# pothosware/PothosComms

Measured on AMD Instinct MI355X. Metric: Msamples/s complex_float32 255-tap FIR, higher is better.
Workload: dtype f32

## Files before the change

### pothoscomms_amd/csrc/fft4096.hpp

```cpp
#pragma once
#include <hip/hip_runtime.h>

namespace pcx {
namespace fft4k {

constexpr int N = 4096;
constexpr int T = 256;
constexpr int LDS_DATA = N + N / 16;
constexpr int LDS_TW2 = 15 * 16;
constexpr int LDS_ELEMS = LDS_DATA + LDS_TW2;
constexpr int TW_TABLE_ELEMS = 15 * 16 + 15 * 256;

typedef float cf __attribute__((ext_vector_type(2)));

__device__ __forceinline__ void cmul2(cf &a, cf &b, cf wa, cf wb)
{
    cf ra, rb;
    asm("v_pk_mul_f32 %0, %2, %4 op_sel:[1,1] op_sel_hi:[0,1] neg_lo:[0,1]\n\t"
        "v_pk_mul_f32 %1, %3, %5 op_sel:[1,1] op_sel_hi:[0,1] neg_lo:[0,1]\n\t"
        "v_pk_fma_f32 %0, %2, %4, %0 op_sel:[0,0,0] op_sel_hi:[1,0,1]\n\t"
        "v_pk_fma_f32 %1, %3, %5, %1 op_sel:[0,0,0] op_sel_hi:[1,0,1]"
        : "=&v"(ra), "=&v"(rb)
        : "v"(a), "v"(b), "v"(wa), "v"(wb));
    a = ra;
    b = rb;
}
__device__ __forceinline__ void cmul2_conj(cf &a, cf &b, cf ha, cf hb)
{
    cf ra, rb;
    asm("v_pk_mul_f32 %0, %2, %4 op_sel:[1,1] op_sel_hi:[0,1] neg_lo:[0,1] neg_hi:[0,1]\n\t"
        "v_pk_mul_f32 %1, %3, %5 op_sel:[1,1] op_sel_hi:[0,1] neg_lo:[0,1] neg_hi:[0,1]\n\t"
        "v_pk_fma_f32 %0, %2, %4, %0 op_sel:[0,0,0] op_sel_hi:[1,0,1] neg_hi:[1,0,0]\n\t"
        "v_pk_fma_f32 %1, %3, %5, %1 op_sel:[0,0,0] op_sel_hi:[1,0,1] neg_hi:[1,0,0]"
        : "=&v"(ra), "=&v"(rb)
        : "v"(a), "v"(b), "v"(ha), "v"(hb));
    a = ra;
    b = rb;
}
__device__ __forceinline__ void addsub_mi(cf &p, cf &m, cf a, cf d)
{
    asm("v_pk_add_f32 %0, %2, %3 op_sel:[0,1] op_sel_hi:[1,0] neg_hi:[0,1]\n\t"
        "v_pk_add_f32 %1, %2, %3 op_sel:[0,1] op_sel_hi:[1,0] neg_lo:[0,1]"
        : "=&v"(p), "=&v"(m)
        : "v"(a), "v"(d));
}
__device__ __forceinline__ cf cmul_cs(cf a, float c, float s)
{
    return cf{__builtin_fmaf(a.x, c, a.y * s), __builtin_fmaf(a.y, c, -a.x * s)};
}

__device__ __forceinline__ void fft4(cf &a0, cf &a1, cf &a2, cf &a3)
{
    const cf t0 = a0 + a2, t1 = a0 - a2, t2 = a1 + a3, d = a1 - a3;
    a0 = t0 + t2;
    a2 = t0 - t2;
    addsub_mi(a1, a3, t1, d);
}
__device__ __forceinline__ void fft4_mi2(cf &a0, cf &a1, cf &a2, cf &a3)
{
    cf t0, t1;
    addsub_mi(t0, t1, a0, a2);
    const cf t2 = a1 + a3, d = a1 - a3;
    a0 = t0 + t2;
    a2 = t0 - t2;
    addsub_mi(a1, a3, t1, d);
}

__device__ __forceinline__ void fft4_conj(cf &a0, cf &a1, cf &a2, cf &a3)
{
    const cf t0 = a0 + a2, t1 = a0 - a2, t2 = a1 + a3, d = a1 - a3;
    asm("v_pk_add_f32 %0, %4, %5 neg_hi:[1,1]\n\t"
        "v_pk_add_f32 %1, %4, %5 neg_lo:[0,1] neg_hi:[1,0]\n\t"
        "v_pk_add_f32 %2, %6, %7 op_sel:[0,1] op_sel_hi:[1,0] neg_hi:[1,0]\n\t"
        "v_pk_add_f32 %3, %6, %7 op_sel:[0,1] op_sel_hi:[1,0] neg_lo:[0,1] neg_hi:[1,1]"
        : "=&v"(a0), "=&v"(a2), "=&v"(a1), "=&v"(a3)
        : "v"(t0), "v"(t2), "v"(t1), "v"(d));
}

struct LaneTw {
    cf a[3];
    cf c[12];
};

__device__ __forceinline__ void fft16_inner(cf (&v)[16])
{
#pragma unroll
    for (int n2 = 0; n2 < 4; n2++) fft4(v[n2], v[4 + n2], v[8 + n2], v[12 + n2]);
}
__device__ __forceinline__ void fft16_outer(cf (&v)[16])
{
#pragma unroll
    for (int k1 = 0; k1 < 4; k1++) fft4(v[4 * k1], v[4 * k1 + 1], v[4 * k1 + 2], v[4 * k1 + 3]);
}
__device__ __forceinline__ void fft16_plain(cf (&v)[16])
{
    constexpr float C1 = 0.92387953251128673848f;
    constexpr float S1 = 0.38268343236508978178f;
    constexpr float R2 = 0.70710678118654752440f;
    fft16_inner(v);
    v[4 * 1 + 1] = cmul_cs(v[4 * 1 + 1], C1, S1);
    v[4 * 1 + 2] = cmul_cs(v[4 * 1 + 2], R2, R2);
    v[4 * 1 + 3] = cmul_cs(v[4 * 1 + 3], S1, C1);
    v[4 * 2 + 1] = cmul_cs(v[4 * 2 + 1], R2, R2);
    v[4 * 2 + 3] = cmul_cs(v[4 * 2 + 3], -R2, R2);
    v[4 * 3 + 1] = cmul_cs(v[4 * 3 + 1], S1, C1);
    v[4 * 3 + 2] = cmul_cs(v[4 * 3 + 2], -R2, R2);
    v[4 * 3 + 3] = cmul_cs(v[4 * 3 + 3], -C1, -S1);
    fft4(v[0], v[1], v[2], v[3]);
    fft4(v[4], v[5], v[6], v[7]);
    fft4_mi2(v[8], v[9], v[10], v[11]);
    fft4(v[12], v[13], v[14], v[15]);
}
__device__ __forceinline__ void fft16_tw(cf (&v)[16], const LaneTw &tw)
{
#pragma unroll
    for (int n1 = 1; n1 < 4; n1++) {
        cmul2(v[4 * n1 + 0], v[4 * n1 + 1], tw.a[n1 - 1], tw.a[n1 - 1]);
        cmul2(v[4 * n1 + 2], v[4 * n1 + 3], tw.a[n1 - 1], tw.a[n1 - 1]);
    }
    fft16_inner(v);
#pragma unroll
    for (int n2 = 1; n2 < 4; n2++) {
        cmul2(v[4 * 0 + n2], v[4 * 1 + n2], tw.c[(n2 - 1) * 4 + 0], tw.c[(n2 - 1) * 4 + 1]);
        cmul2(v[4 * 2 + n2], v[4 * 3 + n2], tw.c[(n2 - 1) * 4 + 2], tw.c[(n2 - 1) * 4 + 3]);
    }
    fft16_outer(v);
}
__device__ __forceinline__ void fft16_tw_conj(cf (&v)[16], const LaneTw &tw)
{
#pragma unroll
    for (int n1 = 1; n1 < 4; n1++) {
        cmul2(v[4 * n1 + 0], v[4 * n1 + 1], tw.a[n1 - 1], tw.a[n1 - 1]);
        cmul2(v[4 * n1 + 2], v[4 * n1 + 3], tw.a[n1 - 1], tw.a[n1 - 1]);
    }
    fft16_inner(v);
#pragma unroll
    for (int n2 = 1; n2 < 4; n2++) {
        cmul2(v[4 * 0 + n2], v[4 * 1 + n2], tw.c[(n2 - 1) * 4 + 0], tw.c[(n2 - 1) * 4 + 1]);
        cmul2(v[4 * 2 + n2], v[4 * 3 + n2], tw.c[(n2 - 1) * 4 + 2], tw.c[(n2 - 1) * 4 + 3]);
    }
#pragma unroll
    for (int k1 = 0; k1 < 4; k1++) fft4_conj(v[4 * k1], v[4 * k1 + 1], v[4 * k1 + 2], v[4 * k1 + 3]);
}
__device__ __forceinline__ constexpr int bin_of(int q) { return (q >> 2) + 4 * (q & 3); }

__device__ __forceinline__ void load_pass3_twiddles(LaneTw &t, const float2 *__restrict__ tab, int j)
{
    const cf *tb = reinterpret_cast<const cf *>(tab) + LDS_TW2;
#pragma unroll
    for (int p = 0; p < 3; p++) t.a[p] = tb[p * 256 + j];
#pragma unroll
    for (int p = 0; p < 12; p++) t.c[p] = tb[(3 + p) * 256 + j];
}
__device__ __forceinline__ void stage_pass2_twiddles(cf *lds, const float2 *__restrict__ tab, int j)
{
    if (j < LDS_TW2) lds[LDS_DATA + j] = reinterpret_cast<const cf *>(tab)[j];
}

typedef unsigned int u32x2 __attribute__((ext_vector_type(2)));

__device__ __forceinline__ __amdgpu_buffer_rsrc_t make_rsrc(const void *p, unsigned bytes)
{
    const unsigned long long a = reinterpret_cast<unsigned long long>(p);
    const unsigned lo = __builtin_amdgcn_readfirstlane((unsigned)a);
    const unsigned hi = __builtin_amdgcn_readfirstlane((unsigned)(a >> 32));
    return __builtin_amdgcn_make_buffer_rsrc(reinterpret_cast<void *>(((unsigned long long)hi << 32) | lo), 0,
                                             (int)__builtin_amdgcn_readfirstlane(bytes), 0x00020000);
}
constexpr int kAuxStream = 2;
template <bool CHECKED, int AUX = kAuxStream>
__device__ __forceinline__ void load_frame(cf (&v)[16], __amdgpu_buffer_rsrc_t rs, int j)
{
#pragma unroll
    for (int r = 0; r < 16; r++) {
        const u32x2 t = CHECKED ? __builtin_amdgcn_raw_buffer_load_b64(rs, (j + 256 * r) * 8, 0, AUX)
                                : __builtin_amdgcn_raw_buffer_load_b64(rs, j * 8, 2048 * r, AUX);
        v[r] = cf{__uint_as_float(t.x), __uint_as_float(t.y)};
    }
}
template <int AUX = 0>
__device__ __forceinline__ void store_cf(__amdgpu_buffer_rsrc_t rs, unsigned voff, cf a)
{
    u32x2 t;
    t.x = __float_as_uint(a.x);
    t.y = __float_as_uint(a.y);
    __builtin_amdgcn_raw_buffer_store_b64(t, rs, (int)voff, 0, AUX);
}

__device__ __forceinline__ cf load_cf(__amdgpu_buffer_rsrc_t rs, int voff, int soff)
{
    const u32x2 t = __builtin_amdgcn_raw_buffer_load_b64(rs, voff, soff, 0);
    return cf{__uint_as_float(t.x), __uint_as_float(t.y)};
}
__device__ __forceinline__ void load_pass3_twiddles(LaneTw &t, __amdgpu_buffer_rsrc_t tab, int j)
{
#pragma unroll
    for (int p = 0; p < 3; p++) t.a[p] = load_cf(tab, j * 8, (LDS_TW2 + p * 256) * 8);
#pragma unroll
    for (int p = 0; p < 12; p++) t.c[p] = load_cf(tab, j * 8, (LDS_TW2 + (3 + p) * 256) * 8);
}

__device__ __forceinline__ float fast_atan2f(float y, float x)
{
    const float ax = __builtin_fabsf(x), ay = __builtin_fabsf(y);
    const float mx = __builtin_fmaxf(ax, ay), mn = __builtin_fminf(ax, ay);
    const float t = mx > 0.f ? mn * __builtin_amdgcn_rcpf(mx) : 0.f;
    const float s = t * t;
    float p = 0.006811532657593489f;
    p = __builtin_fmaf(p, s, -0.03360334783792496f);
    p = __builtin_fmaf(p, s, 0.0796225368976593f);
    p = __builtin_fmaf(p, s, -0.1323327124118805f);
    p = __builtin_fmaf(p, s, 0.19807793200016022f);
    p = __builtin_fmaf(p, s, -0.3331736624240875f);
    p = __builtin_fmaf(p, s, 0.9999961256980896f);
    float r = t * p;
    r = ay > ax ? 1.57079632679489661923f - r : r;
    r = (__float_as_uint(x) >> 31) ? 3.14159265358979323846f - r : r;
    return __builtin_copysignf(r, y);
}

__device__ __forceinline__ cf fast_atan2f_x2(cf y, cf x)
{
    const cf ax = {__builtin_fabsf(x.x), __builtin_fabsf(x.y)}, ay = {__builtin_fabsf(y.x), __builtin_fabsf(y.y)};
    const cf mx = {__builtin_fmaxf(ax.x, ay.x), __builtin_fmaxf(ax.y, ay.y)};
    const cf mn = {__builtin_fminf(ax.x, ay.x), __builtin_fminf(ax.y, ay.y)};
    const cf rc = {mx.x > 0.f ? __builtin_amdgcn_rcpf(mx.x) : 0.f, mx.y > 0.f ? __builtin_amdgcn_rcpf(mx.y) : 0.f};
    const cf t = mn * rc;
    const cf s = t * t;
    auto k2 = [](float c) { return cf{c, c}; };
    cf p = k2(0.006811532657593489f);
    p = __builtin_elementwise_fma(p, s, k2(-0.03360334783792496f));
    p = __builtin_elementwise_fma(p, s, k2(0.0796225368976593f));
    p = __builtin_elementwise_fma(p, s, k2(-0.1323327124118805f));
    p = __builtin_elementwise_fma(p, s, k2(0.19807793200016022f));
    p = __builtin_elementwise_fma(p, s, k2(-0.3331736624240875f));
    p = __builtin_elementwise_fma(p, s, k2(0.9999961256980896f));
    cf r = t * p;
    const cf ro = k2(1.57079632679489661923f) - r;
    r = cf{ay.x > ax.x ? ro.x : r.x, ay.y > ax.y ? ro.y : r.y};
    const cf rn = k2(3.14159265358979323846f) - r;
    r = cf{(__float_as_uint(x.x) >> 31) ? rn.x : r.x, (__float_as_uint(x.y) >> 31) ? rn.y : r.y};
    return cf{__builtin_copysignf(r.x, y.x), __builtin_copysignf(r.y, y.y)};
}

__device__ __forceinline__ int padi(int i) { return i + (i >> 4); }
__device__ __forceinline__ cf cmul1(cf a, cf w)
{
    cf t, r;
    asm("v_pk_mul_f32 %0, %2, %3 op_sel:[1,1] op_sel_hi:[0,1] neg_lo:[0,1]\n\t"
        "v_pk_fma_f32 %1, %2, %3, %0 op_sel:[0,0,0] op_sel_hi:[1,0,1]"
        : "=&v"(t), "=&v"(r)
        : "v"(a), "v"(w));
    return r;
}
__device__ __forceinline__ void fft8(cf &a0, cf &a1, cf &a2, cf &a3, cf &a4, cf &a5, cf &a6, cf &a7)
{
    constexpr float R2 = 0.70710678118654752440f;
    cf e0 = a0, e1 = a2, e2 = a4, e3 = a6, o0 = a1, o1 = a3, o2 = a5, o3 = a7;
    fft4(e0, e1, e2, e3);
    fft4(o0, o1, o2, o3);
    const cf w1 = cmul_cs(o1, R2, R2);
    const cf w3 = cmul_cs(o3, -R2, R2);
    cf p2, m2;
    addsub_mi(p2, m2, e2, o2);
    a0 = e0 + o0; a4 = e0 - o0;
    a1 = e1 + w1; a5 = e1 - w1;
    a2 = p2;      a6 = m2;
    a3 = e3 + w3; a7 = e3 - w3;
}

__device__ __forceinline__ void lds_barrier()
{
    __builtin_amdgcn_fence(__ATOMIC_RELEASE, "workgroup", "local");
    __builtin_amdgcn_s_barrier();
    __builtin_amdgcn_fence(__ATOMIC_ACQUIRE, "workgroup", "local");
}

template <int PART = 0>
__device__ __forceinline__ void pass1_math(cf (&v)[16])
{
    if (PART != 2) fft16_plain(v);
}
template <int PART = 0>
__device__ __forceinline__ void pass1_exchange(cf (&v)[16], cf *lds, int j)
{
    if (PART == 1) return;
    lds_barrier();
#pragma unroll
    for (int q = 0; q < 16; q++) lds[17 * j + bin_of(q)] = v[q];
}
template <int PART = 0>
__device__ __forceinline__ void pass1(cf (&v)[16], cf *lds, int j)
{
    pass1_math<PART>(v);
    pass1_exchange<PART>(v, lds, j);
}
template <int PART = 0>
__device__ __forceinline__ void pass2(cf (&v)[16], cf *lds, int j)
{
    if (PART != 1) {
        lds_barrier();
        const int rb = j + (j >> 4);
#pragma unroll
        for (int r = 0; r < 16; r++) v[r] = lds[rb + 272 * r];
    }
    LaneTw tw;
    const cf *t2 = lds + LDS_DATA + (j & 15);
#pragma unroll
    for (int p = 0; p < 3; p++) tw.a[p] = t2[p * 16];
#pragma unroll
    for (int p = 0; p < 12; p++) tw.c[p] = t2[(3 + p) * 16];
    if (PART != 2) fft16_tw(v, tw);
    else v[0] = v[0] + tw.a[0] + tw.c[0];
    if (PART == 1) return;
    lds_barrier();
    const int wb = (j >> 4) * 272 + (j & 15);
#pragma unroll
    for (int q = 0; q < 16; q++) lds[wb + 17 * bin_of(q)] = v[q];
}
template <int PART = 0, bool CONJ = false>
__device__ __forceinline__ void pass3(cf (&v)[16], const cf *lds, int j, const LaneTw &tw3)
{
    if (PART != 1) {
        lds_barrier();
        const int rb = j + (j >> 4);
#pragma unroll
        for (int r = 0; r < 16; r++) v[r] = lds[rb + 272 * r];
    }
    if (PART != 2) {
        if (CONJ) fft16_tw_conj(v, tw3);
        else fft16_tw(v, tw3);
    }
}

__device__ __forceinline__ void fft16_post(cf (&v)[16], const LaneTw &tw)
{
    fft16_inner(v);
#pragma unroll
    for (int k1 = 1; k1 < 4; k1++) {
        cmul2(v[4 * k1 + 0], v[4 * k1 + 1], tw.c[(k1 - 1) * 4 + 0], tw.c[(k1 - 1) * 4 + 1]);
        cmul2(v[4 * k1 + 2], v[4 * k1 + 3], tw.c[(k1 - 1) * 4 + 2], tw.c[(k1 - 1) * 4 + 3]);
    }
    fft16_outer(v);
#pragma unroll
    for (int k2 = 1; k2 < 4; k2++) {
        cmul2(v[4 * 0 + k2], v[4 * 1 + k2], tw.a[k2 - 1], tw.a[k2 - 1]);
        cmul2(v[4 * 2 + k2], v[4 * 3 + k2], tw.a[k2 - 1], tw.a[k2 - 1]);
    }
}
__device__ __forceinline__ void wave_lds_order()
{
    __builtin_amdgcn_fence(__ATOMIC_RELEASE, "wavefront", "local");
    __builtin_amdgcn_wave_barrier();
    __builtin_amdgcn_fence(__ATOMIC_ACQUIRE, "wavefront", "local");
}
__device__ __forceinline__ int spec_lane(int j) { return (j >> 4) + 16 * (j & 15); }
struct SpectrumLoad {
    cf row[16];
    cf tw2;
};
__device__ __forceinline__ void spectrum_request(SpectrumLoad &t, const float2 *__restrict__ spec, const float2 *__restrict__ twtab, int j)
{
    const __amdgpu_buffer_rsrc_t rs = make_rsrc(spec, N * 8);
#pragma unroll
    for (int k = 0; k < 16; k++) t.row[k] = load_cf(rs, j * 8, 2048 * k);
    t.tw2 = load_cf(make_rsrc(twtab, LDS_TW2 * 8), j * 8, 0);
}
__device__ __forceinline__ void spectrum_turn(cf (&H)[16], const SpectrumLoad &t, cf *lds, int j)
{
#pragma unroll
    for (int k = 0; k < 16; k++) lds[j + 272 * k] = t.row[k];
    if (j < LDS_TW2) lds[LDS_DATA + j] = t.tw2;
    lds_barrier();
#pragma unroll
    for (int k = 0; k < 16; k++) H[k] = lds[spec_lane(j) + 272 * k];
}
__device__ __forceinline__ void load_spectrum_lanes(cf (&H)[16], const float2 *__restrict__ spec, const float2 *__restrict__ twtab, cf *lds, int j)
{
    SpectrumLoad t;
    spectrum_request(t, spec, twtab, j);
    spectrum_turn(H, t, lds, j);
}
__device__ __forceinline__ void load_pass2_twiddles(LaneTw &tw, const cf *lds, int j)
{
    const cf *t2 = lds + LDS_DATA + (j & 15);
#pragma unroll
    for (int p = 0; p < 3; p++) tw.a[p] = t2[p * 16];
#pragma unroll
    for (int p = 0; p < 12; p++) tw.c[p] = t2[(3 + p) * 16];
}
__device__ __forceinline__ void dif_a_math(cf (&v)[16], const LaneTw &tw3) { fft16_post(v, tw3); }
struct NoHook { __device__ __forceinline__ void operator()() const {} };
template <typename HOOK = NoHook>
__device__ __forceinline__ void dif_rest(cf (&v)[16], cf *lds, int j, HOOK before_last = HOOK())
{
    const int row = 272 * (j >> 4), l = j & 15;
    lds_barrier();
#pragma unroll
    for (int q = 0; q < 16; q++) lds[j + 272 * bin_of(q)] = v[q];
    lds_barrier();
#pragma unroll
    for (int r = 0; r < 16; r++) v[r] = lds[row + l + 16 * r];
    LaneTw tw2;
    load_pass2_twiddles(tw2, lds, j);
    fft16_post(v, tw2);
    wave_lds_order();
#pragma unroll
    for (int q = 0; q < 16; q++) lds[row + l + 17 * bin_of(q)] = v[q];
    wave_lds_order();
#pragma unroll
    for (int r = 0; r < 16; r++) v[r] = lds[row + 17 * l + r];
    before_last();
    fft16_plain(v);
}
template <bool CONJ = true>
__device__ __forceinline__ void dit_back(cf (&u)[16], cf *lds, int j, const LaneTw &tw3)
{
    const int row = 272 * (j >> 4), l = j & 15;
    fft16_plain(u);
    wave_lds_order();
#pragma unroll
    for (int q = 0; q < 16; q++) lds[row + 17 * l + bin_of(q)] = u[q];
    wave_lds_order();
#pragma unroll
    for (int r = 0; r < 16; r++) u[r] = lds[row + l + 17 * r];
    LaneTw tw2;
    load_pass2_twiddles(tw2, lds, j);
    fft16_tw(u, tw2);
    wave_lds_order();
#pragma unroll
    for (int q = 0; q < 16; q++) lds[row + l + 16 * bin_of(q)] = u[q];
    lds_barrier();
#pragma unroll
    for (int r = 0; r < 16; r++) u[r] = lds[j + 272 * r];
    if (CONJ) fft16_tw_conj(u, tw3);
    else fft16_tw(u, tw3);
}

}
}
```

### pothoscomms_amd/csrc/fir_ols.hip

```cpp
#include "fft4096.hpp"
#include "ols_block.hpp"
#include "ols_geometry.hpp"
#include "pcx_sched.hpp"
#include <cstdio>
#include <cstdlib>

#include <type_traits>

#include "pcx_internal.hpp"

namespace pcx {

template <bool PREFETCH, int LAUX = 0, int SAUX = 0, int CHUNKED = 0, int DIAG = 0, bool HGLOBAL = false, bool GATED = false, int XCH = 0>
__global__ __launch_bounds__(256, (PREFETCH && !HGLOBAL) ? 3 : 4) void fir_cf32_ols4096_kernel(const float2 *__restrict__ in, size_t in_elems,
                                                                  float2 *__restrict__ out, size_t n_out,
                                                                  const float2 *__restrict__ Hspec, int Kov, int pad,
                                                                  const float2 *__restrict__ twtab, size_t first_full,
                                                                  size_t nfull, size_t nblocks, SchedState *__restrict__ sched, Gate gate)
{
    using namespace fft4k;
    __shared__ cf lds[LDS_ELEMS];
    const int j = threadIdx.x;
    const size_t S = (size_t)(N - Kov);
    size_t b, bend, bstep;
    __shared__ unsigned sched_slot;
    BlockDealer deal;
    if (CHUNKED == 3) {
        static_assert(CHUNKED != 3 || !PREFETCH, "the register prefetch needs the next block's index a block early");
        if (!deal.begin(sched, &sched_slot, nblocks, j)) { deal.finish(j); return; }
        b = GATED ? nblocks - 1 - deal.block() : deal.block();
        bend = nblocks; bstep = 0;
    } else if (CHUNKED == 2) {
        const size_t per = (nblocks + 7) / 8, x = blockIdx.x & 7;
        b = x * per + (blockIdx.x >> 3);
        bend = (x + 1) * per < nblocks ? (x + 1) * per : nblocks;
        bstep = gridDim.x >> 3;
    } else if (CHUNKED) {
        const size_t q = nblocks / gridDim.x, rem = nblocks % gridDim.x, w = blockIdx.x;
        b = w * q + (w < rem ? w : rem);
        bend = b + q + (w < rem ? 1 : 0);
        bstep = 1;
    } else {
        b = blockIdx.x; bend = nblocks; bstep = gridDim.x;
    }
    if (b >= bend) return;
    auto fetch = [&](cf (&dst)[16], size_t blk) {
        if (DIAG == 1) blk = first_full;
        if (blk >= first_full && blk < nfull) {
            if (LAUX >= 4) {
                constexpr int NOV = 1 << (LAUX >= 4 ? LAUX - 4 : 0);
                const __amdgpu_buffer_rsrc_t rs = make_rsrc(in + blk * S - pad, N * 8);
#pragma unroll
                for (int r = 0; r < 16; r++) {
                    const u32x2 t = (r < NOV || r >= 16 - NOV) ? __builtin_amdgcn_raw_buffer_load_b64(rs, j * 8, 2048 * r, 0)
                                                               : __builtin_amdgcn_raw_buffer_load_b64(rs, j * 8, 2048 * r, 2);
                    dst[r] = cf{__uint_as_float(t.x), __uint_as_float(t.y)};
                }
            } else {
                load_frame<false, LAUX>(dst, make_rsrc(in + blk * S - pad, N * 8), j);
            }
        } else {
            const size_t shift = blk * S >= (size_t)pad ? 0 : (size_t)pad - blk * S;
            const size_t first = blk * S + shift - pad;
            const size_t left = in_elems > first ? in_elems - first : 0;
            const size_t want = (size_t)N - shift;
            const __amdgpu_buffer_rsrc_t rs = make_rsrc(in + first, (unsigned)((left < want ? left : want) * 8));
#pragma unroll
            for (int r = 0; r < 16; r++) {
                const u32x2 t = __builtin_amdgcn_raw_buffer_load_b64(rs, (j + 256 * r - (int)shift) * 8, 0, LAUX >= 4 ? 0 : LAUX);
                dst[r] = cf{__uint_as_float(t.x), __uint_as_float(t.y)};
            }
        }
    };
    cf v[16];
    LaneTw tw3;
    cf H[16];
    if (XCH) {
        SpectrumLoad sl;
        spectrum_request(sl, Hspec, twtab, j);
        if (!PREFETCH) {
            if (CHUNKED == 3 && GATED && b < gate.blocks) gate_wait(gate, j);
            fetch(v, b);
        }
        load_pass3_twiddles(tw3, make_rsrc(twtab, TW_TABLE_ELEMS * 8), j);
        spectrum_turn(H, sl, lds, j);
    } else {
        load_pass3_twiddles(tw3, twtab, j);
        stage_pass2_twiddles(lds, twtab, j);
    }
    if (!HGLOBAL && !XCH) {
#pragma unroll
        for (int k = 0; k < 16; k++) H[k] = reinterpret_cast<const cf *>(Hspec)[j + 256 * k];
    }
    static_assert(!XCH || (DIAG == 0 && !HGLOBAL), "the sixteen-lane exchange is built for the product configuration only");
    cf nx[16];
    if (PREFETCH) fetch(nx, b);
    for (; b < bend; b += bstep) {
        if (PREFETCH) {
#pragma unroll
            for (int r = 0; r < 16; r++) v[r] = nx[r];
            const size_t bn = b + bstep;
            if (bn < bend) fetch(nx, bn);
        } else if (XCH) {
        } else {
            if (CHUNKED == 3 && GATED && b < gate.blocks) gate_wait(gate, j);
            fetch(v, b);
        }
        constexpr int PART = DIAG == 3 ? 1 : DIAG == 4 ? 2 : 0;
        if (XCH) dif_a_math(v, tw3);
        else if (DIAG != 2) pass1_math<PART>(v);
        if (CHUNKED == 3) deal.draw(j);
        if (XCH) dif_rest(v, lds, j);
        else if (DIAG != 2) {
        pass1_exchange<PART>(v, lds, j);
        pass2<PART>(v, lds, j);
        pass3<PART>(v, lds, j, tw3);
        }
        cf u[16];
        if (HGLOBAL) {
            const cf *Hp = reinterpret_cast<const cf *>(Hspec);
            asm volatile("" : "+s"(Hp));
#pragma unroll
            for (int k = 0; k < 16; k++) H[k] = Hp[j + 256 * k];
        }
        spectrum_times_h(u, v, H);
        if (CHUNKED == 3) deal.publish(j);
        __builtin_amdgcn_s_setprio(1);
        if (XCH) dit_back(u, lds, j, tw3);
        else if (DIAG != 2) {
        pass1<PART>(u, lds, j);
        pass2<PART>(u, lds, j);
        pass3<PART, true>(u, lds, j, tw3);
        }
        const size_t bo = DIAG == 1 ? 0 : b;
        const size_t room = n_out - bo * S;
        const __amdgpu_buffer_rsrc_t ws = make_rsrc(out + bo * S, (unsigned)((room < S ? room : S) * 8));
        const unsigned vbase = (unsigned)(j - Kov) * 8u;
#pragma unroll
        for (int q = 0; q < 16; q++) {
            const int row = 256 * bin_of(q);
            if (row + 255 < Kov) continue;
            store_cf<SAUX>(ws, vbase + (unsigned)row * 8u, DIAG == 2 ? cf{u[q].x, -u[q].y} : u[q]);
        }
        __builtin_amdgcn_s_setprio(0);
        if (CHUNKED == 3) {
            if (!deal.advance()) break;
            b = GATED ? nblocks - 1 - deal.block() : deal.block();
        }
        if (XCH && !PREFETCH) {
            const size_t bn = CHUNKED == 3 ? b : b + bstep;
            if (bn < bend) {
                if (CHUNKED == 3 && GATED && bn < gate.blocks) gate_wait(gate, j);
                fetch(v, bn);
            }
        }
    }
    if (CHUNKED == 3) deal.finish(j);
}

int launch_fir_cf32_ols4096(const void *in, size_t in_elems, void *out, size_t n_out, const void *Hspec, size_t K,
                            const void *tw4096, void *sched, hipStream_t st, const void *gate_word, unsigned gate_value, int *gated,
                            unsigned slots, size_t lead_valid)
{
    if (gated) *gated = 0;
    if (n_out == 0) return PCX_OK;
    if (K < 1 || K > 2049) { set_error("fir ols: K=%zu outside 1..2049", K); return PCX_ERR_UNSUPPORTED; }
    const int variant = (int)PCX_ENV_INT("PCX_OLS_VARIANT", -1);
    const int align = (int)PCX_ENV_INT("PCX_OLS_ALIGN", 1);
#ifdef PCX_DIAG
    if (variant == 10 || variant == 11 || variant == 12 || variant == 13 || variant == 15 || variant == 16) {
        static bool warned = false;
        if (!warned) fprintf(stderr, "pcx(diag): PCX_OLS_VARIANT=%d selects a TIMING-ONLY build of the overlap-save FIR: its outputs are wrong\n", variant);
        warned = true;
    }
#endif
    const OlsGeometry g = ols_geometry(K, align ? 16 : 1, 4096, n_out, in_elems, lead_valid);
    const size_t Kov = g.Kov, pad = g.pad, nblocks = g.nblocks, first_full = g.first_full, nfull = g.nfull;
    const float2 *pi = (const float2 *)in, *ph = (const float2 *)Hspec, *pt = (const float2 *)tw4096;
    float2 *po = (float2 *)out;
    const bool host_grid = slots > 0 && slots < 128;
    if (!host_grid && (slots < 128 || slots > 1024 || slots % 128)) slots = 1024;
    const long env_static = PCX_ENV_INT("PCX_OLS_SLOTS", 0);
    const unsigned static_slots = env_static > 0 ? (unsigned)env_static : slots;
    const unsigned g4 = persistent_grid(nblocks, static_slots), g3 = persistent_grid(nblocks, 768);
    const unsigned gx = 8 * persistent_grid((nblocks + 7) / 8, 128);
    const bool dealt = !host_grid && sched && nblocks > 2 * (size_t)slots && !PCX_ENV_SET("PCX_SCHED_STATIC");
    if (gate_word && !dealt) return PCX_OK;
    const Gate gate{dealt ? (const unsigned *)gate_word : nullptr, gate_value, 1u};
    if (gated && gate.word) *gated = 1;
#define PCX_OLS_LAUNCH(KERN, GRID) hipLaunchKernelGGL(KERN, dim3(GRID), dim3(256), 0, st, pi, in_elems, po, n_out, ph, (int)Kov, (int)pad, pt, first_full, nfull, nblocks, (SchedState *)sched, gate)
#ifdef PCX_DIAG
    switch (variant) {
    case 0: PCX_OLS_LAUNCH((fir_cf32_ols4096_kernel<true>), g3); goto launched;
    case 1: PCX_OLS_LAUNCH((fir_cf32_ols4096_kernel<false>), g4); goto launched;
    case 2: PCX_OLS_LAUNCH((fir_cf32_ols4096_kernel<false, 2, 0>), g4); goto launched;
    case 3: PCX_OLS_LAUNCH((fir_cf32_ols4096_kernel<false, 2, 2>), g4); goto launched;
    case 4: PCX_OLS_LAUNCH((fir_cf32_ols4096_kernel<false, 0, 0, 1>), g4); goto launched;
    case 5: PCX_OLS_LAUNCH((fir_cf32_ols4096_kernel<true, 0, 0, 0, 0, true>), g4); goto launched;
    case 6: PCX_OLS_LAUNCH((fir_cf32_ols4096_kernel<false, 0, 2>), g4); goto launched;
    case 7: PCX_OLS_LAUNCH((fir_cf32_ols4096_kernel<false, 4, 0>), g4); goto launched;
    case 9: PCX_OLS_LAUNCH((fir_cf32_ols4096_kernel<true, 4, 2>), g3); goto launched;
    case 14: PCX_OLS_LAUNCH((fir_cf32_ols4096_kernel<false, 4, 2, 2>), gx); goto launched;
    case 20: PCX_OLS_LAUNCH((fir_cf32_ols4096_kernel<false, 4, 2>), rounds_grid(nblocks, 1024, 3)); goto launched;
    case 21: PCX_OLS_LAUNCH((fir_cf32_ols4096_kernel<false, 4, 2, 0, 0, true>), rounds_grid(nblocks, 1024, 3)); goto launched;
    case 15: PCX_OLS_LAUNCH((fir_cf32_ols4096_kernel<false, 4, 2, 0, 3>), g4); goto launched;
    case 16: PCX_OLS_LAUNCH((fir_cf32_ols4096_kernel<false, 4, 2, 0, 4>), g4); goto launched;
    case 12: PCX_OLS_LAUNCH((fir_cf32_ols4096_kernel<false, 4, 2, 0, 1>), g4); goto launched;
    case 13: PCX_OLS_LAUNCH((fir_cf32_ols4096_kernel<false, 4, 2, 0, 2>), g4); goto launched;
    case 30: PCX_OLS_LAUNCH((fir_cf32_ols4096_kernel<false, 4, 0, 3, 0, false, false, 1>), g4); goto launched;
    case 31: PCX_OLS_LAUNCH((fir_cf32_ols4096_kernel<false, 4, 3, 3, 0, false, false, 1>), g4); goto launched;
    case 32: PCX_OLS_LAUNCH((fir_cf32_ols4096_kernel<false, 4, 18, 3, 0, false, false, 1>), g4); goto launched;
    case 33: PCX_OLS_LAUNCH((fir_cf32_ols4096_kernel<false, 4, 19, 3, 0, false, false, 1>), g4); goto launched;
    case 34: PCX_OLS_LAUNCH((fir_cf32_ols4096_kernel<false, 4, 16, 3, 0, false, false, 1>), g4); goto launched;
    case 35: PCX_OLS_LAUNCH((fir_cf32_ols4096_kernel<false, 4, 17, 3, 0, false, false, 1>), g4); goto launched;
    case 10: PCX_OLS_LAUNCH((fir_cf32_ols4096_kernel<false, 0, 0, 0, 1>), g4); goto launched;
    case 11: PCX_OLS_LAUNCH((fir_cf32_ols4096_kernel<false, 0, 0, 0, 2>), g4); goto launched;
    default: break;
    }
#else
    (void)variant; (void)g3; (void)gx;
#endif
    if (dealt && gate.word) {
        const long env_gd = PCX_ENV_INT("PCX_GATED_SLOTS", 0);
        const unsigned gd = env_gd > 0 ? (unsigned)env_gd : slots;
        if (Kov <= 256) PCX_OLS_LAUNCH((fir_cf32_ols4096_kernel<false, 4, 2, 3, 0, false, true, 1>), gd);
        else if (Kov <= 512) PCX_OLS_LAUNCH((fir_cf32_ols4096_kernel<false, 5, 2, 3, 0, false, true, 1>), gd);
        else if (Kov <= 1024) PCX_OLS_LAUNCH((fir_cf32_ols4096_kernel<false, 6, 2, 3, 0, false, true, 1>), gd);
        else PCX_OLS_LAUNCH((fir_cf32_ols4096_kernel<false, 0, 2, 3, 0, false, true, 1>), gd);
    } else if (dealt) {
        const long env_gd = PCX_ENV_INT("PCX_DEALT_SLOTS", 0);
        const unsigned gd = env_gd > 0 ? (unsigned)env_gd : slots;
#ifdef PCX_DIAG
        if (PCX_ENV_INT("PCX_OLS_XCH", 1) == 0) {
            if (Kov <= 256) PCX_OLS_LAUNCH((fir_cf32_ols4096_kernel<false, 4, 2, 3>), gd);
            else PCX_OLS_LAUNCH((fir_cf32_ols4096_kernel<false, 0, 2, 3>), gd);
        } else
#endif
        if (Kov <= 256) PCX_OLS_LAUNCH((fir_cf32_ols4096_kernel<false, 4, 2, 3, 0, false, false, 1>), gd);
        else if (Kov <= 512) PCX_OLS_LAUNCH((fir_cf32_ols4096_kernel<false, 5, 2, 3, 0, false, false, 1>), gd);
        else if (Kov <= 1024) PCX_OLS_LAUNCH((fir_cf32_ols4096_kernel<false, 6, 2, 3, 0, false, false, 1>), gd);
        else PCX_OLS_LAUNCH((fir_cf32_ols4096_kernel<false, 0, 2, 3, 0, false, false, 1>), gd);
    }
    else if (Kov <= 256) PCX_OLS_LAUNCH((fir_cf32_ols4096_kernel<false, 4, 2, 0, 0, false, false, 1>), g4);
    else if (Kov <= 512) PCX_OLS_LAUNCH((fir_cf32_ols4096_kernel<false, 5, 2, 0, 0, false, false, 1>), g4);
    else if (Kov <= 1024) PCX_OLS_LAUNCH((fir_cf32_ols4096_kernel<false, 6, 2, 0, 0, false, false, 1>), g4);
    else PCX_OLS_LAUNCH((fir_cf32_ols4096_kernel<false, 0, 2, 0, 0, false, false, 1>), g4);
#ifdef PCX_DIAG
launched:
#endif
#undef PCX_OLS_LAUNCH
    PCX_LAUNCH_CHECK();
    return PCX_OK;
}

template <int NOV, bool DYN = false>
__global__ __launch_bounds__(256, 4) void fir_f32_ols4096_kernel(const float *__restrict__ in, size_t in_elems,
                                                                 float *__restrict__ out, size_t n_out,
                                                                 const float2 *__restrict__ Hspec, int Kov, int pad,
                                                                 const float2 *__restrict__ twtab, size_t nblocks, SchedState *__restrict__ sched)
{
    using namespace fft4k;
    __shared__ cf lds[LDS_ELEMS];
    const int j = threadIdx.x;
    const size_t S = (size_t)(N - Kov);
    const size_t npairs = (nblocks + 1) / 2;
    __shared__ unsigned sched_slot;
    BlockWalk<DYN> walk;
    if (!walk.begin(sched, &sched_slot, npairs, j)) { walk.finish(j); return; }
    LaneTw tw3;
    load_pass3_twiddles(tw3, make_rsrc(twtab, TW_TABLE_ELEMS * 8), j);
    cf H[16];
    load_spectrum_lanes(H, Hspec, twtab, lds, j);
    for (;;) {
        const size_t p = walk.block();
        const size_t bA = 2 * p, bB = 2 * p + 1;
        cf v[16];
        if (bA > 0 && bB * S - pad + N <= in_elems) {
            const __amdgpu_buffer_rsrc_t ra = make_rsrc(in + bA * S - pad, N * 4);
            const __amdgpu_buffer_rsrc_t rb = make_rsrc(in + bB * S - pad, N * 4);
#pragma unroll
            for (int r = 0; r < 16; r++) {
                unsigned a, b;
                if (r < NOV || r >= 16 - NOV) {
                    a = __builtin_amdgcn_raw_buffer_load_b32(ra, j * 4, 1024 * r, 0);
                    b = __builtin_amdgcn_raw_buffer_load_b32(rb, j * 4, 1024 * r, 0);
                } else {
                    a = __builtin_amdgcn_raw_buffer_load_b32(ra, j * 4, 1024 * r, 2);
                    b = __builtin_amdgcn_raw_buffer_load_b32(rb, j * 4, 1024 * r, 2);
                }
                v[r] = cf{__uint_as_float(a), __uint_as_float(b)};
            }
        } else {
            const size_t shiftA = bA * S >= (size_t)pad ? 0 : (size_t)pad - bA * S;
            const size_t firstA = bA * S + shiftA - pad;
            const size_t leftA = in_elems > firstA ? in_elems - firstA : 0;
            const size_t wantA = (size_t)N - shiftA;
            const bool haveB = bB < nblocks;
            const size_t firstB = haveB ? bB * S - pad : 0;
            const size_t leftB = haveB && in_elems > firstB ? in_elems - firstB : 0;
            const __amdgpu_buffer_rsrc_t ra = make_rsrc(in + firstA, (unsigned)((leftA < wantA ? leftA : wantA) * 4));
            const __amdgpu_buffer_rsrc_t rb = make_rsrc(in + firstB, (unsigned)((leftB < (size_t)N ? leftB : (size_t)N) * 4));
#pragma unroll
            for (int r = 0; r < 16; r++) {
                const unsigned a = __builtin_amdgcn_raw_buffer_load_b32(ra, (j + 256 * r - (int)shiftA) * 4, 0, 0);
                const unsigned b = __builtin_amdgcn_raw_buffer_load_b32(rb, (j + 256 * r) * 4, 0, 0);
                v[r] = cf{__uint_as_float(a), __uint_as_float(b)};
            }
        }
        dif_a_math(v, tw3);
        walk.draw(j);
        dif_rest(v, lds, j);
        cf u[16];
        spectrum_times_h(u, v, H);
        walk.publish(j);
        __builtin_amdgcn_s_setprio(1);
        dit_back(u, lds, j, tw3);
        const size_t roomA = n_out - bA * S;
        const size_t roomB = bB < nblocks ? n_out - bB * S : 0;
        const __amdgpu_buffer_rsrc_t wa = make_rsrc(out + bA * S, (unsigned)((roomA < S ? roomA : S) * 4));
        const __amdgpu_buffer_rsrc_t wb = make_rsrc(out + (bB < nblocks ? bB * S : 0), (unsigned)((roomB < S ? roomB : S) * 4));
        const unsigned vbase = (unsigned)(j - Kov) * 4u;
#pragma unroll
        for (int q = 0; q < 16; q++) {
            const int row = 256 * bin_of(q);
            if (row + 255 < Kov) continue;
            __builtin_amdgcn_raw_buffer_store_b32(__float_as_uint(u[q].x), wa, (int)(vbase + (unsigned)row * 4u), 0, 2);
            __builtin_amdgcn_raw_buffer_store_b32(__float_as_uint(u[q].y), wb, (int)(vbase + (unsigned)row * 4u), 0, 2);
        }
        __builtin_amdgcn_s_setprio(0);
        if (!walk.advance()) break;
    }
    walk.finish(j);
}

int launch_fir_f32_ols4096(const void *in, size_t in_elems, void *out, size_t n_out, const void *Hspec, size_t K,
                           const void *tw4096, void *sched, hipStream_t st)
{
    if (n_out == 0) return PCX_OK;
    if (K < 1 || K > 2049) { set_error("fir ols (real): K=%zu outside 1..2049", K); return PCX_ERR_UNSUPPORTED; }
    const OlsGeometry g = ols_geometry(K, 32, 4096, n_out, in_elems, 0);
    const size_t Kov = g.Kov, pad = g.pad, nblocks = g.nblocks;
    const size_t npairs = (nblocks + 1) / 2;
    const bool dyn = sched && npairs > 2 * 1024 && !PCX_ENV_SET("PCX_SCHED_STATIC");
    const unsigned grid = dyn ? 1024u : persistent_grid(npairs, 1024);
#define PCX_REAL_LAUNCH(NOV)                                                                                                                  \
    do {                                                                                                                                      \
        if (dyn) hipLaunchKernelGGL((fir_f32_ols4096_kernel<NOV, true>), dim3(grid), dim3(256), 0, st, (const float *)in, in_elems, (float *)out, n_out, \
                                    (const float2 *)Hspec, (int)Kov, (int)pad, (const float2 *)tw4096, nblocks, (SchedState *)sched);            \
        else hipLaunchKernelGGL((fir_f32_ols4096_kernel<NOV, false>), dim3(grid), dim3(256), 0, st, (const float *)in, in_elems, (float *)out, n_out,    \
                                (const float2 *)Hspec, (int)Kov, (int)pad, (const float2 *)tw4096, nblocks, (SchedState *)nullptr);              \
    } while (0)
    if (Kov <= 256) PCX_REAL_LAUNCH(1);
    else if (Kov <= 512) PCX_REAL_LAUNCH(2);
    else if (Kov <= 1024) PCX_REAL_LAUNCH(4);
    else PCX_REAL_LAUNCH(8);
#undef PCX_REAL_LAUNCH
    PCX_LAUNCH_CHECK();
    return PCX_OK;
}

__global__ __launch_bounds__(256, 4) void fir_cf32_ols4096_poly_kernel(const float2 *__restrict__ in, size_t in_elems,
                                                                       float2 *__restrict__ out, size_t n_iter,
                                                                       const float2 *__restrict__ Hspec, int Km1,
                                                                       const float2 *__restrict__ twtab, size_t nblocks,
                                                                       unsigned L, unsigned M, unsigned jrow, unsigned long long magic)
{
    using namespace fft4k;
    __shared__ cf lds[LDS_ELEMS];
    const int j = threadIdx.x;
    const size_t S = (size_t)(N - Km1);
    size_t b = blockIdx.x;
    if (b >= nblocks) return;
    LaneTw tw3;
    load_pass3_twiddles(tw3, make_rsrc(twtab, TW_TABLE_ELEMS * 8), j);
    cf H[16];
    load_spectrum_lanes(H, Hspec, twtab, lds, j);
    for (; b < nblocks; b += gridDim.x) {
        cf v[16];
        {
            const size_t left = in_elems - b * S;
            if (left >= (size_t)N) load_frame<false, 0>(v, make_rsrc(in + b * S, N * 8), j);
            else load_frame<true, 0>(v, make_rsrc(in + b * S, (unsigned)(left * 8)), j);
        }
        dif_a_math(v, tw3);
        dif_rest(v, lds, j);
        cf u[16];
        spectrum_times_h(u, v, H);
        dit_back(u, lds, j, tw3);
        const unsigned long long B0 = (unsigned long long)(b * S) * L + jrow + 1;
        const unsigned long long q0 = B0 / M;
        const unsigned r0 = (unsigned)(B0 - q0 * M);
        const size_t n_left = n_iter - b * S;
        const unsigned nl = n_left < (size_t)N ? (unsigned)n_left : (unsigned)N;
        float2 *ob = out + q0 - 1;
        asm volatile("" : "+s"(ob));
#pragma unroll
        for (int q = 0; q < 16; q++) {
            const int row = 256 * bin_of(q);
            if (row + 255 < Km1) continue;
// ... 254 lines not shown
```

Baseline: 348,300.

## Hand-schedule LDS reads with staged lgkmcnt waits in FFT exchange passes

Adds an LDSX path that issues all per-pass LDS row and twiddle reads as inline ds_read_b64 with immediate offsets. Each read is waited on with a graded s_waitcnt lgkmcnt, so butterflies on the first rows start while later rows are still arriving. Twiddle loads are interleaved with the complex multiplies, and the barrier at the top of dif_rest is dropped by hoisting a single barrier after the spectrum staging. The path is on by default for every launch branch. It relies on the compiler not inserting other LDS or scalar ops between the manual issues and their waits, which could silently break correctness, and it may raise register pressure.

```diff
diff --git a/pothoscomms_amd/csrc/fft4096.hpp b/pothoscomms_amd/csrc/fft4096.hpp
--- a/pothoscomms_amd/csrc/fft4096.hpp
+++ b/pothoscomms_amd/csrc/fft4096.hpp
@@ -1,5 +1,7 @@
 #pragma once
 #include <hip/hip_runtime.h>
+#include <type_traits>
+#include <utility>
 
 namespace pcx {
 namespace fft4k {
@@ -92,12 +94,11 @@
 #pragma unroll
     for (int k1 = 0; k1 < 4; k1++) fft4(v[4 * k1], v[4 * k1 + 1], v[4 * k1 + 2], v[4 * k1 + 3]);
 }
-__device__ __forceinline__ void fft16_plain(cf (&v)[16])
+__device__ __forceinline__ void fft16_plain_rest(cf (&v)[16])
 {
     constexpr float C1 = 0.92387953251128673848f;
     constexpr float S1 = 0.38268343236508978178f;
     constexpr float R2 = 0.70710678118654752440f;
-    fft16_inner(v);
     v[4 * 1 + 1] = cmul_cs(v[4 * 1 + 1], C1, S1);
     v[4 * 1 + 2] = cmul_cs(v[4 * 1 + 2], R2, R2);
     v[4 * 1 + 3] = cmul_cs(v[4 * 1 + 3], S1, C1);
@@ -110,6 +111,11 @@
     fft4(v[4], v[5], v[6], v[7]);
     fft4_mi2(v[8], v[9], v[10], v[11]);
     fft4(v[12], v[13], v[14], v[15]);
+}
+__device__ __forceinline__ void fft16_plain(cf (&v)[16])
+{
+    fft16_inner(v);
+    fft16_plain_rest(v);
 }
 __device__ __forceinline__ void fft16_tw(cf (&v)[16], const LaneTw &tw)
 {
@@ -389,16 +395,153 @@
 #pragma unroll
     for (int p = 0; p < 12; p++) tw.c[p] = t2[(3 + p) * 16];
 }
+__device__ __forceinline__ unsigned lds_byte_addr(const cf *p)
+{
+    return (unsigned)(size_t)(const __attribute__((address_space(3))) cf *)p;
+}
+template <int OFF>
+__device__ __forceinline__ void issue_read(cf &d, unsigned addr)
+{
+    static_assert(OFF >= 0 && OFF < 65536, "ds offset field: 16 bits");
+    asm volatile("ds_read_b64 %0, %1 offset:%2" : "=v"(d) : "v"(addr), "i"(OFF) : "memory");
+}
+typedef std::integer_sequence<int, 0, 4, 8, 12, 1, 5, 9, 13, 2, 6, 10, 14, 3, 7, 11, 15> RowsInnerFirst;
+typedef std::integer_sequence<int, 4, 5, 6, 7, 8, 9, 10, 11, 12, 13, 14, 15, 0, 1, 2, 3> RowsOuterFirst;
+template <int STRIDE_BYTES, int... R>
+__device__ __forceinline__ void issue_rows(cf (&v)[16], unsigned addr, std::integer_sequence<int, R...>)
+{
+    (issue_read<STRIDE_BYTES * R>(v[R], addr), ...);
+}
+__device__ __forceinline__ void issue_tw_a(LaneTw &tw, unsigned t2)
+{
+    issue_read<(LDS_DATA + 0 * 16) * 8>(tw.a[0], t2);
+    issue_read<(LDS_DATA + 1 * 16) * 8>(tw.a[1], t2);
+    issue_read<(LDS_DATA + 2 * 16) * 8>(tw.a[2], t2);
+}
+template <int G>
+__device__ __forceinline__ void issue_tw_c(LaneTw &tw, unsigned t2)
+{
+    issue_read<(LDS_DATA + (3 + 4 * G) * 16) * 8>(tw.c[4 * G + 0], t2);
+    issue_read<(LDS_DATA + (4 + 4 * G) * 16) * 8>(tw.c[4 * G + 1], t2);
+    issue_read<(LDS_DATA + (5 + 4 * G) * 16) * 8>(tw.c[4 * G + 2], t2);
+    issue_read<(LDS_DATA + (6 + 4 * G) * 16) * 8>(tw.c[4 * G + 3], t2);
+}
+template <int YOUNGER>
+__device__ __forceinline__ void landed(cf &a, cf &b, cf &c)
+{
+    asm volatile("s_waitcnt lgkmcnt(%3)" : "+v"(a), "+v"(b), "+v"(c) : "i"(YOUNGER) : "memory");
+}
+template <int YOUNGER>
+__device__ __forceinline__ void landed(cf &a, cf &b, cf &c, cf &d)
+{
+    asm volatile("s_waitcnt lgkmcnt(%4)" : "+v"(a), "+v"(b), "+v"(c), "+v"(d) : "i"(YOUNGER) : "memory");
+}
+template <int YOUNGER>
+__device__ __forceinline__ void landed(cf &a, cf &b, cf &c, cf &d, cf &e, cf &f, cf &g, cf &h)
+{
+    asm volatile("s_waitcnt lgkmcnt(%8)" : "+v"(a), "+v"(b), "+v"(c), "+v"(d), "+v"(e), "+v"(f), "+v"(g), "+v"(h) : "i"(YOUNGER) : "memory");
+}
+__device__ __forceinline__ void fft16_inner_landing(cf (&v)[16])
+{
+    landed<12>(v[0], v[4], v[8], v[12]);
+    fft4(v[0], v[4], v[8], v[12]);
+    landed<8>(v[1], v[5], v[9], v[13], v[0], v[4], v[8], v[12]);
+    fft4(v[1], v[5], v[9], v[13]);
+    landed<4>(v[2], v[6], v[10], v[14], v[1], v[5], v[9], v[13]);
+    fft4(v[2], v[6], v[10], v[14]);
+    landed<0>(v[3], v[7], v[11], v[15], v[2], v[6], v[10], v[14]);
+    fft4(v[3], v[7], v[11], v[15]);
+}
+__device__ __forceinline__ void fft16_post_landing(cf (&v)[16], LaneTw &tw, unsigned t2)
+{
+    landed<15>(tw.c[0], tw.c[1], tw.c[2], tw.c[3], tw.c[4], tw.c[5], tw.c[6], tw.c[7]);
+    fft16_inner_landing(v);
+    cmul2(v[4], v[5], tw.c[0], tw.c[1]);
+    cmul2(v[6], v[7], tw.c[2], tw.c[3]);
+    issue_tw_c<2>(tw, t2);
+    cmul2(v[8], v[9], tw.c[4], tw.c[5]);
+    cmul2(v[10], v[11], tw.c[6], tw.c[7]);
+    issue_tw_a(tw, t2);
+    landed<3>(tw.c[8], tw.c[9], tw.c[10], tw.c[11], v[8], v[9], v[10], v[11]);
+    cmul2(v[12], v[13], tw.c[8], tw.c[9]);
+    cmul2(v[14], v[15], tw.c[10], tw.c[11]);
+    fft16_outer(v);
+    landed<0>(tw.a[0], tw.a[1], tw.a[2]);
+#pragma unroll
+    for (int k2 = 1; k2 < 4; k2++) {
+        cmul2(v[4 * 0 + k2], v[4 * 1 + k2], tw.a[k2 - 1], tw.a[k2 - 1]);
+        cmul2(v[4 * 2 + k2], v[4 * 3 + k2], tw.a[k2 - 1], tw.a[k2 - 1]);
+    }
+}
+__device__ __forceinline__ void fft16_plain_landing(cf (&v)[16])
+{
+    fft16_inner_landing(v);
+    fft16_plain_rest(v);
+}
+template <bool CONJ, bool T2, typename TW>
+__device__ __forceinline__ void fft16_tw_landing(cf (&v)[16], TW &tw, unsigned t2)
+{
+    landed<12>(v[4], v[5], v[6], v[7]);
+    cmul2(v[4], v[5], tw.a[0], tw.a[0]);
+    cmul2(v[6], v[7], tw.a[0], tw.a[0]);
+    landed<8>(v[8], v[9], v[10], v[11], v[4], v[5], v[6], v[7]);
+    cmul2(v[8], v[9], tw.a[1], tw.a[1]);
+    cmul2(v[10], v[11], tw.a[1], tw.a[1]);
+    landed<4>(v[12], v[13], v[14], v[15], v[8], v[9], v[10], v[11]);
+    cmul2(v[12], v[13], tw.a[2], tw.a[2]);
+    cmul2(v[14], v[15], tw.a[2], tw.a[2]);
+    landed<0>(v[0], v[1], v[2], v[3], v[12], v[13], v[14], v[15]);
+    if constexpr (T2) {
+        issue_tw_c<0>(tw, t2);
+        issue_tw_c<1>(tw, t2);
+    }
+    fft16_inner(v);
+    if constexpr (T2) landed<4>(tw.c[0], tw.c[1], tw.c[2], tw.c[3], v[3], v[7], v[11], v[15]);
+    cmul2(v[1], v[5], tw.c[0], tw.c[1]);
+    cmul2(v[9], v[13], tw.c[2], tw.c[3]);
+    if constexpr (T2) {
+        issue_tw_c<2>(tw, t2);
+        landed<4>(tw.c[4], tw.c[5], tw.c[6], tw.c[7], v[1], v[5], v[9], v[13]);
+    }
+    cmul2(v[2], v[6], tw.c[4], tw.c[5]);
+    cmul2(v[10], v[14], tw.c[6], tw.c[7]);
+    if constexpr (T2) landed<0>(tw.c[8], tw.c[9], tw.c[10], tw.c[11], v[2], v[6], v[10], v[14]);
+    cmul2(v[3], v[7], tw.c[8], tw.c[9]);
+    cmul2(v[11], v[15], tw.c[10], tw.c[11]);
+    if (CONJ) {
+#pragma unroll
+        for (int k1 = 0; k1 < 4; k1++) fft4_conj(v[4 * k1], v[4 * k1 + 1], v[4 * k1 + 2], v[4 * k1 + 3]);
+    } else {
+        fft16_outer(v);
+    }
+}
 __device__ __forceinline__ void dif_a_math(cf (&v)[16], const LaneTw &tw3) { fft16_post(v, tw3); }
 struct NoHook { __device__ __forceinline__ void operator()() const {} };
-template <typename HOOK = NoHook>
+template <int LDSX = 0, typename HOOK = NoHook>
 __device__ __forceinline__ void dif_rest(cf (&v)[16], cf *lds, int j, HOOK before_last = HOOK())
 {
     const int row = 272 * (j >> 4), l = j & 15;
-    lds_barrier();
+    if (!LDSX) lds_barrier();
 #pragma unroll
     for (int q = 0; q < 16; q++) lds[j + 272 * bin_of(q)] = v[q];
     lds_barrier();
+    if constexpr (LDSX != 0) {
+        static_assert(!LDSX || std::is_same<HOOK, NoHook>::value, "nothing may join the counter between the reads and their waits");
+        const unsigned image = lds_byte_addr(lds);
+        const unsigned t2 = image + l * 8;
+        LaneTw tw2;
+        issue_tw_c<0>(tw2, t2);
+        issue_tw_c<1>(tw2, t2);
+        issue_rows<16 * 8>(v, image + (row + l) * 8, RowsInnerFirst());
+        fft16_post_landing(v, tw2, t2);
+        wave_lds_order();
+#pragma unroll
+        for (int q = 0; q < 16; q++) lds[row + l + 17 * bin_of(q)] = v[q];
+        wave_lds_order();
+        issue_rows<8>(v, image + (row + 17 * l) * 8, RowsInnerFirst());
+        fft16_plain_landing(v);
+        return;
+    }
 #pragma unroll
     for (int r = 0; r < 16; r++) v[r] = lds[row + l + 16 * r];
     LaneTw tw2;
@@ -413,7 +556,7 @@
     before_last();
     fft16_plain(v);
 }
-template <bool CONJ = true>
+template <bool CONJ = true, int LDSX = 0>
 __device__ __forceinline__ void dit_back(cf (&u)[16], cf *lds, int j, const LaneTw &tw3)
 {
     const int row = 272 * (j >> 4), l = j & 15;
@@ -422,6 +565,22 @@
 #pragma unroll
     for (int q = 0; q < 16; q++) lds[row + 17 * l + bin_of(q)] = u[q];
     wave_lds_order();
+    if constexpr (LDSX != 0) {
+        const unsigned image = lds_byte_addr(lds);
+        const unsigned t2 = image + l * 8;
+        LaneTw tw2;
+        issue_tw_a(tw2, t2);
+        issue_rows<17 * 8>(u, image + (row + l) * 8, RowsOuterFirst());
+        landed<15>(tw2.a[0], tw2.a[1], tw2.a[2]);
+        fft16_tw_landing<false, true>(u, tw2, t2);
+        wave_lds_order();
+#pragma unroll
+        for (int q = 0; q < 16; q++) lds[row + l + 16 * bin_of(q)] = u[q];
+        lds_barrier();
+        issue_rows<272 * 8>(u, image + j * 8, RowsOuterFirst());
+        fft16_tw_landing<CONJ, false>(u, tw3, 0u);
+        return;
+    }
 #pragma unroll
     for (int r = 0; r < 16; r++) u[r] = lds[row + l + 17 * r];
     LaneTw tw2;
diff --git a/pothoscomms_amd/csrc/fir_ols.hip b/pothoscomms_amd/csrc/fir_ols.hip
--- a/pothoscomms_amd/csrc/fir_ols.hip
+++ b/pothoscomms_amd/csrc/fir_ols.hip
@@ -11,7 +11,7 @@
 
 namespace pcx {
 
-template <bool PREFETCH, int LAUX = 0, int SAUX = 0, int CHUNKED = 0, int DIAG = 0, bool HGLOBAL = false, bool GATED = false, int XCH = 0>
+template <bool PREFETCH, int LAUX = 0, int SAUX = 0, int CHUNKED = 0, int DIAG = 0, bool HGLOBAL = false, bool GATED = false, int XCH = 0, int LDSX = 0>
 __global__ __launch_bounds__(256, (PREFETCH && !HGLOBAL) ? 3 : 4) void fir_cf32_ols4096_kernel(const float2 *__restrict__ in, size_t in_elems,
                                                                   float2 *__restrict__ out, size_t n_out,
                                                                   const float2 *__restrict__ Hspec, int Kov, int pad,
@@ -84,6 +84,7 @@
         }
         load_pass3_twiddles(tw3, make_rsrc(twtab, TW_TABLE_ELEMS * 8), j);
         spectrum_turn(H, sl, lds, j);
+        if (LDSX) lds_barrier();
     } else {
         load_pass3_twiddles(tw3, twtab, j);
         stage_pass2_twiddles(lds, twtab, j);
@@ -93,6 +94,7 @@
         for (int k = 0; k < 16; k++) H[k] = reinterpret_cast<const cf *>(Hspec)[j + 256 * k];
     }
     static_assert(!XCH || (DIAG == 0 && !HGLOBAL), "the sixteen-lane exchange is built for the product configuration only");
+    static_assert(!LDSX || (XCH && !PREFETCH), "LDSX is a spelling of the sixteen-lane exchange");
     cf nx[16];
     if (PREFETCH) fetch(nx, b);
     for (; b < bend; b += bstep) {
@@ -110,7 +112,7 @@
         if (XCH) dif_a_math(v, tw3);
         else if (DIAG != 2) pass1_math<PART>(v);
         if (CHUNKED == 3) deal.draw(j);
-        if (XCH) dif_rest(v, lds, j);
+        if (XCH) dif_rest<LDSX>(v, lds, j);
         else if (DIAG != 2) {
         pass1_exchange<PART>(v, lds, j);
         pass2<PART>(v, lds, j);
@@ -126,7 +128,7 @@
         spectrum_times_h(u, v, H);
         if (CHUNKED == 3) deal.publish(j);
         __builtin_amdgcn_s_setprio(1);
-        if (XCH) dit_back(u, lds, j, tw3);
+        if (XCH) dit_back<true, LDSX>(u, lds, j, tw3);
         else if (DIAG != 2) {
         pass1<PART>(u, lds, j);
         pass2<PART>(u, lds, j);
@@ -188,6 +190,9 @@
     if (gate_word && !dealt) return PCX_OK;
     const Gate gate{dealt ? (const unsigned *)gate_word : nullptr, gate_value, 1u};
     if (gated && gate.word) *gated = 1;
+#ifdef PCX_DIAG
+    const bool ldsx = PCX_ENV_INT("PCX_OLS_LDSX", 1) != 0;
+#endif
 #define PCX_OLS_LAUNCH(KERN, GRID) hipLaunchKernelGGL(KERN, dim3(GRID), dim3(256), 0, st, pi, in_elems, po, n_out, ph, (int)Kov, (int)pad, pt, first_full, nfull, nblocks, (SchedState *)sched, gate)
 #ifdef PCX_DIAG
     switch (variant) {
@@ -220,13 +225,21 @@
 #else
     (void)variant; (void)g3; (void)gx;
 #endif
+#define PCX_OLS_BY_KOV(CH, GATED, XCH, LDSX, GRID)                                                                          \
+    do {                                                                                                                    \
+        if (Kov <= 256) PCX_OLS_LAUNCH((fir_cf32_ols4096_kernel<false, 4, 2, CH, 0, false, GATED, XCH, LDSX>), GRID);       \
+        else if (Kov <= 512) PCX_OLS_LAUNCH((fir_cf32_ols4096_kernel<false, 5, 2, CH, 0, false, GATED, XCH, LDSX>), GRID);  \
+        else if (Kov <= 1024) PCX_OLS_LAUNCH((fir_cf32_ols4096_kernel<false, 6, 2, CH, 0, false, GATED, XCH, LDSX>), GRID); \
+        else PCX_OLS_LAUNCH((fir_cf32_ols4096_kernel<false, 0, 2, CH, 0, false, GATED, XCH, LDSX>), GRID);                  \
+    } while (0)
     if (dealt && gate.word) {
         const long env_gd = PCX_ENV_INT("PCX_GATED_SLOTS", 0);
         const unsigned gd = env_gd > 0 ? (unsigned)env_gd : slots;
-        if (Kov <= 256) PCX_OLS_LAUNCH((fir_cf32_ols4096_kernel<false, 4, 2, 3, 0, false, true, 1>), gd);
-        else if (Kov <= 512) PCX_OLS_LAUNCH((fir_cf32_ols4096_kernel<false, 5, 2, 3, 0, false, true, 1>), gd);
-        else if (Kov <= 1024) PCX_OLS_LAUNCH((fir_cf32_ols4096_kernel<false, 6, 2, 3, 0, false, true, 1>), gd);
-        else PCX_OLS_LAUNCH((fir_cf32_ols4096_kernel<false, 0, 2, 3, 0, false, true, 1>), gd);
+#ifdef PCX_DIAG
+        if (!ldsx) PCX_OLS_BY_KOV(3, true, 1, 0, gd);
+        else
+#endif
+        PCX_OLS_BY_KOV(3, true, 1, 1, gd);
     } else if (dealt) {
         const long env_gd = PCX_ENV_INT("PCX_DEALT_SLOTS", 0);
         const unsigned gd = env_gd > 0 ? (unsigned)env_gd : slots;
@@ -234,17 +247,18 @@
         if (PCX_ENV_INT("PCX_OLS_XCH", 1) == 0) {
             if (Kov <= 256) PCX_OLS_LAUNCH((fir_cf32_ols4096_kernel<false, 4, 2, 3>), gd);
             else PCX_OLS_LAUNCH((fir_cf32_ols4096_kernel<false, 0, 2, 3>), gd);
-        } else
-#endif
-        if (Kov <= 256) PCX_OLS_LAUNCH((fir_cf32_ols4096_kernel<false, 4, 2, 3, 0, false, false, 1>), gd);
-        else if (Kov <= 512) PCX_OLS_LAUNCH((fir_cf32_ols4096_kernel<false, 5, 2, 3, 0, false, false, 1>), gd);
-        else if (Kov <= 1024) PCX_OLS_LAUNCH((fir_cf32_ols4096_kernel<false, 6, 2, 3, 0, false, false, 1>), gd);
-        else PCX_OLS_LAUNCH((fir_cf32_ols4096_kernel<false, 0, 2, 3, 0, false, false, 1>), gd);
-    }
-    else if (Kov <= 256) PCX_OLS_LAUNCH((fir_cf32_ols4096_kernel<false, 4, 2, 0, 0, false, false, 1>), g4);
-    else if (Kov <= 512) PCX_OLS_LAUNCH((fir_cf32_ols4096_kernel<false, 5, 2, 0, 0, false, false, 1>), g4);
-    else if (Kov <= 1024) PCX_OLS_LAUNCH((fir_cf32_ols4096_kernel<false, 6, 2, 0, 0, false, false, 1>), g4);
-    else PCX_OLS_LAUNCH((fir_cf32_ols4096_kernel<false, 0, 2, 0, 0, false, false, 1>), g4);
+        } else if (!ldsx) PCX_OLS_BY_KOV(3, false, 1, 0, gd);
+        else
+#endif
+        PCX_OLS_BY_KOV(3, false, 1, 1, gd);
+    } else {
+#ifdef PCX_DIAG
+        if (!ldsx) PCX_OLS_BY_KOV(0, false, 1, 0, g4);
+        else
+#endif
+        PCX_OLS_BY_KOV(0, false, 1, 1, g4);
+    }
+#undef PCX_OLS_BY_KOV
 #ifdef PCX_DIAG
 launched:
 #endif
```

New measurement: 355,500, median of 4. Within noise of the previous version (+2.1%).
